# lebrice/blurred-GAN

Hardware: AMD Instinct MI355X
Metric: images/sec (G+D+GP step) (higher is better)
Workload: dtype f32; 1 GPU; celeba64 64x64x3 batch 256/GPU, blur sigma 5.0 (31 taps), D-step+GP+G-step+Adam; global_batch=256, parallelism=dp1

## Files before the change

blurred-gan_amd/csrc/conv_rows.hip:

```cpp
#include "conv_common.h"
#include <algorithm>
#include <cstdlib>
#include <cstring>
#include <type_traits>

namespace {

typedef float floatx4 __attribute__((ext_vector_type(4)));

struct RowParams {
  const float* A;
  const float* Wt;
  float* C;
  int B, Hi, Wi, Ck, Ho, Wo, N;
  int pt, pl, flip;
  int R, strips;
  int wpr, ipw;
  int epi_mode;
  const float* bias;
  const float* ref;
  const unsigned char* keep;
  size_t keep_elems;
  float alpha, scale;
};

__device__ inline int floordiv(int a, int b) { return a >= 0 ? a / b : -((-a + b - 1) / b); }

__device__ inline float tanh_branchless(float x) {
  float ax = fabsf(x);
  ax = ax > 15.f ? 15.f : ax;
  const float e = __builtin_amdgcn_exp2f(ax * 2.885390081777927f);
  const float big = 1.f - 2.f * __builtin_amdgcn_rcpf(e + 1.f);
  const float x2 = ax * ax;
  const float small = ax * fmaf(x2, fmaf(x2, fmaf(x2, -17.f / 315.f, 2.f / 15.f), -1.f / 3.f), 1.f);
  return copysignf(ax < 0.1f ? small : big, x);
}

template <int KS, int K, int S, int PIXW, int EP>
__global__ __launch_bounds__(PIXW * 4) void conv_rows_scatter_kernel(const RowParams p) {
  constexpr int NTH = PIXW * 4;
  constexpr unsigned kOob = 0x80000000u;
  extern __shared__ __attribute__((aligned(16))) float row_lds[];
  constexpr int AS = 4 * KS + 4;
  float* abuf = row_lds;
  constexpr int PS = PIXW * 17 + 1;
  float* pbuf = row_lds + 2 * PIXW * AS;
  const int tid = threadIdx.x, lane = tid & 63, wave = tid >> 6;
  const int li = lane & 15, kq = lane >> 4;
  const int t = wave % p.wpr, img = wave / p.wpr;
  const int strip = blockIdx.x % p.strips, bgrp = blockIdx.x / p.strips;
  const int Ck = 4 * KS, N = p.N;
  const int y0 = strip * p.R, y1 = min(y0 + p.R, p.Ho);
  const int iy_lo = -floordiv(-(y0 + p.pt - (K - 1)), S);
  const int iy_hi = floordiv(y1 - 1 + p.pt, S);
  const int nrows = iy_hi - iy_lo + 1;
  const int nimg = min(p.ipw, p.B - bgrp * p.ipw);
  const size_t img0 = (size_t)bgrp * p.ipw;
  const __amdgpu_buffer_rsrc_t rsA = __builtin_amdgcn_make_buffer_rsrc(const_cast<float*>(p.A + img0 * p.Hi * p.Wi * Ck), 0,
                                                                        nimg * p.Hi * p.Wi * Ck * 4, 0x00020000);
  const __amdgpu_buffer_rsrc_t rsC = __builtin_amdgcn_make_buffer_rsrc(p.C + img0 * p.Ho * p.Wo * N, 0, nimg * p.Ho * p.Wo * N * 4, 0x00020000);

  float bw[K][KS];
  {
    const int lc = min(li, K * N - 1);
    const int kw = lc / N, n = lc - kw * N;
#pragma unroll
    for (int kh = 0; kh < K; ++kh) {
      const int tap = p.flip ? (K - 1 - kh) * K + (K - 1 - kw) : kh * K + kw;
#pragma unroll
      for (int ks = 0; ks < KS; ++ks) {
        const float w = p.Wt[((size_t)tap * N + n) * Ck + 4 * ks + kq];
        bw[kh][ks] = li < K * N ? w : 0.f;
      }
    }
  }
  floatx4 acc[K];
#pragma unroll
  for (int i = 0; i < K; ++i) acc[i] = floatx4{0.f, 0.f, 0.f, 0.f};

  constexpr int QPR = KS;
  constexpr int NQ = PIXW * QPR / NTH;
  static_assert(NQ >= 1, "Ck >= 16");
  unsigned g_off[NQ], l_off[NQ];
#pragma unroll
  for (int q = 0; q < NQ; ++q) {
    const int f = tid + q * NTH, pix = f / QPR, c4 = f - pix * QPR;
    const int im = pix / p.Wi, ix = pix - im * p.Wi;
    g_off[q] = im < nimg ? (unsigned)(((im * p.Hi * p.Wi + ix) * Ck + c4 * 4) * 4) : kOob;
    l_off[q] = (unsigned)(pix * AS + c4 * 4);
  }
  const int rowB = p.Wi * Ck * 4;
  auto gload = [&](int r, float4 (&g)[NQ]) {
    const int iy = iy_lo + r;
    const bool row_ok = r < nrows && (unsigned)iy < (unsigned)p.Hi;
    const unsigned add = row_ok ? (unsigned)(iy * rowB) : 0u, force = row_ok ? 0u : kOob;
#pragma unroll
    for (int q = 0; q < NQ; ++q)
      g[q] = __builtin_bit_cast(float4, __builtin_amdgcn_raw_buffer_load_b128(rsA, (g_off[q] + add) | force, 0, 0));
  };
  auto lstore = [&](int buf, const float4 (&g)[NQ]) {
#pragma unroll
    for (int q = 0; q < NQ; ++q) *reinterpret_cast<float4*>(abuf + (size_t)buf * PIXW * AS + l_off[q]) = g[q];
  };
  const float* afrag = abuf + ((size_t)img * p.Wi + 16 * t + li) * AS + kq;
  constexpr int NE = (S * (16 / K) + 3) / 4;
  constexpr int NTERM = (K + S - 1) / S;
  int e_src[NE][NTERM];
  unsigned e_dst[NE];
  float e_bias[NE], e_mul[NE];
  int e_n[NE];
  if (tid < 2 * S) pbuf[(size_t)tid * PS + PIXW * 17] = 0.f;
  {
    const int per_img = p.Wo * N;
#pragma unroll
    for (int q = 0; q < NE; ++q) {
      const int e = tid + q * NTH;
      const int im = e / per_img, rem = e - im * per_img;
      const int x = rem / N, n = rem - x * N;
      const bool ok = e < p.ipw * per_img && im < nimg;
      e_dst[q] = ok ? (unsigned)(((im * p.Ho * p.Wo + x) * N + n) * 4) : kOob;
      e_n[q] = n;
      e_bias[q] = ok && p.bias ? p.bias[n] : 0.f;
      e_mul[q] = ok && p.epi_mode == BG_EPI_AFFINE_LRELU ? p.ref[n] : 0.f;
#pragma unroll
      for (int i = 0; i < NTERM; ++i) {
        const int kw = (x + p.pl) % S + i * S;
        const int num = x + p.pl - kw, ix = num / S;
        e_src[q][i] = (ok && kw < K && num >= 0 && ix < p.Wi) ? (im * p.Wi + ix) * 17 + kw * N + n : PIXW * 17;
      }
    }
  }
  const size_t out0 = img0 * p.Ho * p.Wo * N;
  auto pwrite = [&](const floatx4& pacc, int slot) {
    float* pb = pbuf + (size_t)slot * PS;
#pragma unroll
    for (int rr = 0; rr < 4; ++rr) pb[((size_t)img * p.Wi + 16 * t + 4 * kq + rr) * 17 + li] = pacc[rr];
  };
  auto pstore = [&](int slot, int y, bool live) {
    const float* pb = pbuf + (size_t)slot * PS;
    float v[NE];
#pragma unroll
    for (int q = 0; q < NE; ++q) {
      v[q] = pb[e_src[q][0]];
#pragma unroll
      for (int i = 1; i < NTERM; ++i) v[q] += pb[e_src[q][i]];
    }
    const unsigned add = live ? (unsigned)(y * p.Wo * N * 4) : 0u, force = live ? 0u : kOob;
#pragma unroll
    for (int q = 0; q < NE; ++q) {
      const unsigned off = (e_dst[q] + add) | force;
      float o;
      if (EP == 0) {
        o = v[q] + e_bias[q];
      } else if (EP == 1) {
        o = tanh_branchless(v[q] + e_bias[q]);
      } else {
        const bool mine = (off & kOob) == 0;
        o = mine ? bg::apply_epilogue_pre(p, v[q], out0 + (off >> 2), e_bias[q], e_mul[q]) : 0.f;
      }
      __builtin_amdgcn_raw_buffer_store_b32(__builtin_bit_cast(unsigned, o), rsC, off, 0, 0);
    }
  };

  float4 g0[NQ], g1[NQ], g2[NQ], g3[NQ];
  gload(0, g0);
  gload(1, g1);
  gload(2, g2);
  gload(3, g3);
  lstore(0, g0);
  gload(4, g0);
#pragma unroll
  for (int i = 0; i < 4 * NE * S; ++i) __builtin_amdgcn_raw_buffer_store_b32(0u, rsC, kOob + 4u * i, 0, 0);
  int y_prev = 0;
  bool have_prev = false;
  auto flush_prev = [&](int prev_par) {
#pragma unroll
    for (int kh = 0; kh < S; ++kh) {
      const int y = y_prev + kh;
      pstore(prev_par * S + kh, y, have_prev & (y >= y0) & (y < y1));
    }
  };
  auto trip = [&](int r, auto parity, float4 (&g)[NQ]) {
    constexpr int cur = decltype(parity)::value;
    __syncthreads();
    float a[KS];
#pragma unroll
    for (int ks = 0; ks < KS; ++ks) a[ks] = afrag[(size_t)cur * PIXW * AS + 4 * ks];
#pragma unroll
    for (int ks = 0; ks < KS; ++ks)
#pragma unroll
      for (int kh = 0; kh < K; ++kh) acc[kh] = __builtin_amdgcn_mfma_f32_16x16x4f32(a[ks], bw[kh][ks], acc[kh], 0, 0, 0);
    flush_prev(cur ^ 1);
    lstore(cur ^ 1, g);
    gload(r + 5, g);
#pragma unroll
    for (int kh = 0; kh < S; ++kh) pwrite(acc[kh], cur * S + kh);
    y_prev = (iy_lo + r) * S - p.pt;
    have_prev = true;
#pragma unroll
    for (int i = 0; i < K; ++i) acc[i] = i + S < K ? acc[i + S] : floatx4{0.f, 0.f, 0.f, 0.f};
  };
  int r = 0;
  for (; r + 4 <= nrows; r += 4) {
    trip(r, std::integral_constant<int, 0>{}, g1);
    trip(r + 1, std::integral_constant<int, 1>{}, g2);
    trip(r + 2, std::integral_constant<int, 0>{}, g3);
    trip(r + 3, std::integral_constant<int, 1>{}, g0);
  }
  int last_par = 1;
  if (r < nrows) {
    trip(r, std::integral_constant<int, 0>{}, g1);
    last_par = 0;
    if (r + 1 < nrows) {
      trip(r + 1, std::integral_constant<int, 1>{}, g2);
      last_par = 1;
      if (r + 2 < nrows) {
        trip(r + 2, std::integral_constant<int, 0>{}, g3);
        last_par = 0;
      }
    }
  }
  __syncthreads();
  if (last_par == 0) flush_prev(0); else flush_prev(1);
}

template <int K, int S>
int launch_rows(const RowParams& p, dim3 grid, size_t lds, hipStream_t s) {
  const bool wide = p.Wi == 128;
  const int ep = p.epi_mode == BG_EPI_NONE ? 0 : p.epi_mode == BG_EPI_TANH ? 1 : 2;
#define BG_RS2(KSv, EPv) do { if (wide) bg::launch((conv_rows_scatter_kernel<KSv, K, S, 128, EPv>), grid, dim3(512), lds, s, p); \
                              else bg::launch((conv_rows_scatter_kernel<KSv, K, S, 64, EPv>), grid, dim3(256), lds, s, p); } while (0)
#define BG_RS(KSv) do { if (ep == 0) BG_RS2(KSv, 0); else if (ep == 1) BG_RS2(KSv, 1); else BG_RS2(KSv, 2); } while (0)
  switch (p.Ck) {
    case 16: BG_RS(4); return 1;
    case 32: BG_RS(8); return 1;
    case 64: BG_RS(16); return 1;
    default: return 0;
  }
#undef BG_RS
#undef BG_RS2
}

constexpr int kRgHalo = 16;

struct RowGParams {
  const float* A;
  const float* Wt;
  float* C;
  int B, Hi, Wi, Ct, Ho, Wo, N;
  int s, pt, pl, flip;
  int R, strips;
  int epi_mode;
  const float* bias;
  const float* ref;
  const unsigned char* keep;
  size_t keep_elems;
  float alpha, scale;
};

template <int TG, int NT, int K, bool MASK>
__global__ __launch_bounds__(256) void conv_rows_gather_kernel(const RowGParams p) {
  extern __shared__ __attribute__((aligned(16))) float xl[];
  const int tid = threadIdx.x, lane = tid & 63, wave = tid >> 6;
  const int li = lane & 15, kq = lane >> 4;
  const int Ct = p.Ct, N = 16 * NT, st = p.s;
  const int RS = p.Wi * Ct + 2 * kRgHalo;
  const int strip = blockIdx.x % p.strips, b = blockIdx.x / p.strips;
  const int oy0 = strip * p.R, rows = min(p.R, p.Ho - oy0);
  const int nrows_in = (rows - 1) * st + K;

  float bw[K][4][NT];
#pragma unroll
  for (int ks = 0; ks < 4; ++ks) {
    const int i = 4 * ks + kq, kw = i / Ct, ci = i - kw * Ct;
#pragma unroll
    for (int kh = 0; kh < K; ++kh) {
      const int tap = p.flip ? (K - 1 - kh) * K + (K - 1 - kw) : kh * K + kw;
#pragma unroll
      for (int nt = 0; nt < NT; ++nt) bw[kh][ks][nt] = i < K * Ct ? p.Wt[((size_t)tap * N + nt * 16 + li) * Ct + ci] : 0.f;
    }
  }
  const int RL = p.Wi * Ct;
  if ((RL & 3) == 0) {
    const int q4 = RS / 4;
    bg::stage_rows_f4<4>(xl, nrows_in, q4, RS, tid, [&](int r, int c4) -> const float* {
      const int iy = oy0 * st - p.pt + r, e = c4 * 4 - kRgHalo;
      return ((unsigned)iy < (unsigned)p.Hi && (unsigned)e < (unsigned)RL) ? p.A + ((size_t)b * p.Hi + iy) * RL + e : nullptr;
    });
  } else {
    for (int idx = tid; idx < nrows_in * RS; idx += 256) {
      const int r = idx / RS, c = idx - r * RS;
      const int iy = oy0 * st - p.pt + r, e = c - kRgHalo;
      float v = 0.f;
      if ((unsigned)iy < (unsigned)p.Hi && (unsigned)e < (unsigned)RL) v = p.A[((size_t)b * p.Hi + iy) * RL + e];
      xl[idx] = v;
    }
  }
  __syncthreads();

  float e_bias[NT], e_mul[NT];
#pragma unroll
  for (int nt = 0; nt < NT; ++nt) {
    e_bias[nt] = p.bias ? p.bias[nt * 16 + li] : 0.f;
    e_mul[nt] = p.epi_mode == BG_EPI_AFFINE_LRELU ? p.ref[nt * 16 + li] : 1.f;
  }
  const int groups = p.Wo / (16 * TG);
  const int nunits = rows * groups;
  for (int u = wave; u < nunits; u += 4) {
    const int r = u / groups, g = u - r * groups;
    const int oy = oy0 + r, ox0 = g * 16 * TG;
    floatx4 acc[TG][NT];
#pragma unroll
    for (int tg = 0; tg < TG; ++tg)
#pragma unroll
      for (int nt = 0; nt < NT; ++nt) acc[tg][nt] = floatx4{0.f, 0.f, 0.f, 0.f};
    const float* abase = xl + (size_t)(r * st) * RS + kRgHalo + ((ox0 + li) * st - p.pl) * Ct + kq;
#pragma unroll
    for (int kh = 0; kh < K; ++kh) {
      float a[TG][4];
#pragma unroll
      for (int tg = 0; tg < TG; ++tg)
#pragma unroll
        for (int ks = 0; ks < 4; ++ks) a[tg][ks] = abase[(size_t)kh * RS + tg * 16 * st * Ct + 4 * ks];
#pragma unroll
      for (int ks = 0; ks < 4; ++ks)
#pragma unroll
        for (int tg = 0; tg < TG; ++tg)
#pragma unroll
          for (int nt = 0; nt < NT; ++nt) acc[tg][nt] = __builtin_amdgcn_mfma_f32_16x16x4f32(a[tg][ks], bw[kh][ks][nt], acc[tg][nt], 0, 0, 0);
    }
    constexpr bool mask_epi = MASK;
#pragma unroll
    for (int tg = 0; tg < TG; ++tg) {
      const size_t pix0 = ((size_t)b * p.Ho + oy) * p.Wo + ox0 + 16 * tg + 4 * kq;
      unsigned char e_keep[4][NT];
      if (mask_epi) {
#pragma unroll
        for (int rr = 0; rr < 4; ++rr)
#pragma unroll
          for (int nt = 0; nt < NT; ++nt) {
            const size_t idx = (pix0 + rr) * N + nt * 16 + li;
            e_keep[rr][nt] = p.keep[(p.keep_elems == 0 || idx < p.keep_elems) ? idx : 0];
          }
      }
#pragma unroll
      for (int rr = 0; rr < 4; ++rr)
#pragma unroll
        for (int nt = 0; nt < NT; ++nt) {
          const size_t idx = (pix0 + rr) * N + nt * 16 + li;
          if (mask_epi) {
            float v = acc[tg][nt][rr] + e_bias[nt];
            v = v > 0.f ? v : p.alpha * v;
            if (p.keep_elems == 0 || idx < p.keep_elems) v = e_keep[rr][nt] ? v * p.scale : 0.f;
            p.C[idx] = v;
          } else {
            p.C[idx] = bg::apply_epilogue_pre(p, acc[tg][nt][rr], idx, e_bias[nt], e_mul[nt]);
          }
        }
    }
  }
}

template <int K>
int launch_rows_gather(const RowGParams& p, int tg, dim3 grid, size_t lds, hipStream_t s) {
  const int nt = p.N / 16;
  const bool mask = p.epi_mode == BG_EPI_BIAS_LRELU && p.keep != nullptr;
#define BG_RG(TGv, NTv) do { if (mask) bg::launch((conv_rows_gather_kernel<TGv, NTv, K, true>), grid, dim3(256), lds, s, p); \
                             else bg::launch((conv_rows_gather_kernel<TGv, NTv, K, false>), grid, dim3(256), lds, s, p); } while (0)
  if (tg == 1) { if (nt == 1) BG_RG(1, 1); else if (nt == 2) BG_RG(1, 2); else BG_RG(1, 4); }
  else if (tg == 2) { if (nt == 1) BG_RG(2, 1); else if (nt == 2) BG_RG(2, 2); else BG_RG(2, 4); }
  else { if (nt == 1) BG_RG(4, 1); else if (nt == 2) BG_RG(4, 2); else BG_RG(4, 4); }
#undef BG_RG
  return 1;
}

}

namespace bg {

int try_conv_rows_gather(int bwd_data, const float* a, const float* w, float* c, int B, int H, int W, int Cin, int Cout, int k, int s,
                         const bg_epilogue* epi, void* stream, int* taken) {
  *taken = 0;
  static const int off = getenv("BG_NO_ROWS") ? 1 : 0;
  if (off || (k != 5 && k != 3)) return BG_OK;
  RowGParams p;
  memset(&p, 0, sizeof p);
  int Ho, Wo, pt, pl;
  same_pads(H, k, s, &Ho, &pt);
  same_pads(W, k, s, &Wo, &pl);
  if (bwd_data) {
    if (s != 1 || Cout * k > 16 || (Cin != 16 && Cin != 32 && Cin != 64)) return BG_OK;
    p.Hi = H; p.Wi = W; p.Ct = Cout; p.Ho = H; p.Wo = W; p.N = Cin; p.s = 1; p.pt = k - 1 - pt; p.pl = k - 1 - pl; p.flip = 1;
  } else {
    if (Cin * k > 16 || (Cout != 16 && Cout != 32 && Cout != 64)) return BG_OK;
    p.Hi = H; p.Wi = W; p.Ct = Cin; p.Ho = Ho; p.Wo = Wo; p.N = Cout; p.s = s; p.pt = pt; p.pl = pl; p.flip = 0;
  }
  if (p.Wo % 16 != 0) return BG_OK;
  if ((size_t)B * p.Ho * p.Wo * p.N >= (1ull << 31)) return BG_OK;
  const int tiles = p.Wo / 16;
  const int tg = tiles % 4 == 0 ? 4 : (tiles % 2 == 0 ? 2 : 1);
  p.A = a; p.Wt = w; p.C = c; p.B = B;
  static const int rows_r = getenv("BG_ROWSG_R") ? atoi(getenv("BG_ROWSG_R")) : 0;
  p.R = std::min(rows_r ? rows_r : (s == 2 ? 8 : 16), p.Ho);
  p.strips = (int)cdiv(p.Ho, p.R);
  const size_t lds = ((size_t)((p.R - 1) * p.s + k) * (p.Wi * p.Ct + 2 * kRgHalo)) * sizeof(float);
  if (lds > 64 * 1024) return BG_OK;
  p.epi_mode = BG_EPI_NONE; p.alpha = 0.3f; p.scale = 1.f;
  if (epi) {
    BG_REQUIRE(epi->mode >= BG_EPI_NONE && epi->mode <= BG_EPI_AFFINE_LRELU, BG_ERR_UNSUPPORTED, "conv rows: epilogue mode %d", epi->mode);
    BG_REQUIRE(epi->mode != BG_EPI_MUL_GRAD || epi->ref, BG_ERR_NULL, "conv rows: BG_EPI_MUL_GRAD needs ref");
    BG_REQUIRE(epi->mode != BG_EPI_AFFINE_LRELU || (epi->ref && epi->bias), BG_ERR_NULL, "conv rows: BG_EPI_AFFINE_LRELU needs ref and bias");
    p.epi_mode = epi->mode; p.bias = epi->bias; p.ref = epi->ref; p.keep = epi->keep; p.keep_elems = epi->keep_elems; p.alpha = epi->alpha; p.scale = epi->scale;
  }
  const dim3 grid((unsigned)(B * p.strips));
  const double flops = 2.0 * B * (double)Ho * Wo * Cin * Cout * k * k;
  Launch L(stream, bwd_data ? "conv_rows_thin_k_dgrad" : "conv_rows_thin_k_fwd", flops, 0);
  if (k == 5) launch_rows_gather<5>(p, tg, grid, lds, L.s);
  else launch_rows_gather<3>(p, tg, grid, lds, L.s);
  *taken = 1;
  return L.done("conv_rows_gather_kernel");
}



int try_conv_rows(int bwd_data, const float* a, const float* w, float* c, int B, int H, int W, int Cin, int Cout, int k, int s,
                  const bg_epilogue* epi, void* stream, int* taken) {
  *taken = 0;
  static const int off = getenv("BG_NO_ROWS") ? 1 : 0;
  if (off || (k != 5 && k != 3)) return BG_OK;
  RowParams p;
  memset(&p, 0, sizeof p);
  int Ho, Wo, pt, pl;
  same_pads(H, k, s, &Ho, &pt);
  same_pads(W, k, s, &Wo, &pl);
  if (bwd_data) {
    if (Cin * k > 16 || (Cout != 16 && Cout != 32 && Cout != 64)) return BG_OK;
    p.Hi = Ho; p.Wi = Wo; p.Ck = Cout; p.Ho = H; p.Wo = W; p.N = Cin; p.pt = pt; p.pl = pl; p.flip = 0;
  } else {
    if (s != 1 || Cout * k > 16 || (Cin != 16 && Cin != 32 && Cin != 64)) return BG_OK;
    p.Hi = H; p.Wi = W; p.Ck = Cin; p.Ho = H; p.Wo = W; p.N = Cout; p.pt = k - 1 - pt; p.pl = k - 1 - pl; p.flip = 1;
  }
  if (p.Wi != 16 && p.Wi != 32 && p.Wi != 64 && p.Wi != 128) return BG_OK;
  if ((size_t)B * p.Hi * p.Wi * p.Ck >= (1ull << 31) || (size_t)B * p.Ho * p.Wo * p.N >= (1ull << 31)) return BG_OK;
  p.A = a; p.Wt = w; p.C = c; p.B = B;
  static const int rows_r = getenv("BG_ROWS_R") ? atoi(getenv("BG_ROWS_R")) : 0;
  p.R = std::min(rows_r ? rows_r : (s == 1 ? 32 : 16), p.Ho);
  p.strips = (int)cdiv(p.Ho, p.R);
  p.wpr = p.Wi / 16;
  p.ipw = p.Wi == 128 ? 1 : 4 / p.wpr;
  const int pixw = p.Wi == 128 ? 128 : 64;
  if ((long)p.ipw * p.Wo * p.N > (long)((s * (16 / k) + 3) / 4) * pixw * 4) return BG_OK;
  if ((size_t)p.ipw * p.Hi * p.Wi * p.Ck >= (1ull << 29) || (size_t)p.ipw * p.Ho * p.Wo * p.N >= (1ull << 29)) return BG_OK;
  p.epi_mode = BG_EPI_NONE; p.alpha = 0.3f; p.scale = 1.f;
  if (epi) {
    BG_REQUIRE(epi->mode >= BG_EPI_NONE && epi->mode <= BG_EPI_AFFINE_LRELU, BG_ERR_UNSUPPORTED, "conv rows: epilogue mode %d", epi->mode);
    BG_REQUIRE(epi->mode != BG_EPI_MUL_GRAD || epi->ref, BG_ERR_NULL, "conv rows: BG_EPI_MUL_GRAD needs ref");
    BG_REQUIRE(epi->mode != BG_EPI_AFFINE_LRELU || (epi->ref && epi->bias), BG_ERR_NULL, "conv rows: BG_EPI_AFFINE_LRELU needs ref and bias");
    p.epi_mode = epi->mode; p.bias = epi->bias; p.ref = epi->ref; p.keep = epi->keep; p.keep_elems = epi->keep_elems; p.alpha = epi->alpha; p.scale = epi->scale;
  }
  const dim3 grid((unsigned)(cdiv(B, p.ipw) * p.strips));
  const size_t lds = ((size_t)2 * pixw * (p.Ck + 4) + (size_t)2 * s * (pixw * 17 + 1)) * sizeof(float);
  const double flops = 2.0 * B * (double)H * W * Cin * Cout * k * k / (s * s);
  Launch L(stream, bwd_data ? "conv_rows_dgrad" : "conv_rows_fwd", flops, 0);
  int ok;
  if (k == 5) ok = s == 2 ? launch_rows<5, 2>(p, grid, lds, L.s) : launch_rows<5, 1>(p, grid, lds, L.s);
  else ok = s == 2 ? launch_rows<3, 2>(p, grid, lds, L.s) : launch_rows<3, 1>(p, grid, lds, L.s);
  (void)ok;
  *taken = 1;
  return L.done("conv_rows_scatter_kernel");
}

}
```

Baseline: 32460 images/s.

## Make thin-K row-gather conv persistent with double-buffered register prefetch

Turns the row-gather conv kernel into a persistent kernel sized to a few workgroups per CU. It prefetches the next strip's input rows into registers via buffer loads and stashes them into a second LDS buffer while the current strip computes. It also swaps the MFMA operand order so each lane holds four consecutive channels, which allows float4 epilogue stores and uchar4 keep-mask loads. The cost is doubled LDS, smaller default strips, added alignment requirements and register pressure from the prefetch arrays.

```diff
diff --git a/blurred-gan_amd/csrc/conv_rows.hip b/blurred-gan_amd/csrc/conv_rows.hip
--- a/blurred-gan_amd/csrc/conv_rows.hip
+++ b/blurred-gan_amd/csrc/conv_rows.hip
@@ -242,6 +242,8 @@
 }
 
 constexpr int kRgHalo = 16;
+constexpr int kRgPF = 6;
+constexpr int kRgWgPerCu = 3;
 
 struct RowGParams {
   const float* A;
@@ -250,6 +252,9 @@
   int B, Hi, Wi, Ct, Ho, Wo, N;
   int s, pt, pl, flip;
   int R, strips;
+  int units;
+  int vec;
+  unsigned a_bytes;
   int epi_mode;
   const float* bias;
   const float* ref;
@@ -261,13 +266,15 @@
 template <int TG, int NT, int K, bool MASK>
 __global__ __launch_bounds__(256) void conv_rows_gather_kernel(const RowGParams p) {
   extern __shared__ __attribute__((aligned(16))) float xl[];
+  constexpr unsigned kOob = 0x80000000u;
   const int tid = threadIdx.x, lane = tid & 63, wave = tid >> 6;
   const int li = lane & 15, kq = lane >> 4;
   const int Ct = p.Ct, N = 16 * NT, st = p.s;
-  const int RS = p.Wi * Ct + 2 * kRgHalo;
-  const int strip = blockIdx.x % p.strips, b = blockIdx.x / p.strips;
-  const int oy0 = strip * p.R, rows = min(p.R, p.Ho - oy0);
-  const int nrows_in = (rows - 1) * st + K;
+  const int RL = p.Wi * Ct;
+  const int RS = RL + 2 * kRgHalo;
+  const int nrows_in = (p.R - 1) * st + K;
+  const int BUF = nrows_in * RS;
+  const __amdgpu_buffer_rsrc_t rsA = __builtin_amdgcn_make_buffer_rsrc(const_cast<float*>(p.A), 0, (int)p.a_bytes, 0x00020000);
 
   float bw[K][4][NT];
 #pragma unroll
@@ -280,84 +287,140 @@
       for (int nt = 0; nt < NT; ++nt) bw[kh][ks][nt] = i < K * Ct ? p.Wt[((size_t)tap * N + nt * 16 + li) * Ct + ci] : 0.f;
     }
   }
-  const int RL = p.Wi * Ct;
-  if ((RL & 3) == 0) {
-    const int q4 = RS / 4;
-    bg::stage_rows_f4<4>(xl, nrows_in, q4, RS, tid, [&](int r, int c4) -> const float* {
-      const int iy = oy0 * st - p.pt + r, e = c4 * 4 - kRgHalo;
-      return ((unsigned)iy < (unsigned)p.Hi && (unsigned)e < (unsigned)RL) ? p.A + ((size_t)b * p.Hi + iy) * RL + e : nullptr;
-    });
-  } else {
-    for (int idx = tid; idx < nrows_in * RS; idx += 256) {
-      const int r = idx / RS, c = idx - r * RS;
-      const int iy = oy0 * st - p.pt + r, e = c - kRgHalo;
-      float v = 0.f;
-      if ((unsigned)iy < (unsigned)p.Hi && (unsigned)e < (unsigned)RL) v = p.A[((size_t)b * p.Hi + iy) * RL + e];
-      xl[idx] = v;
-    }
-  }
+  for (int i = tid; i < 2 * nrows_in * 2 * kRgHalo; i += 256) {
+    const int row = i / (2 * kRgHalo), e = i - row * (2 * kRgHalo);
+    xl[(size_t)row * RS + (e < kRgHalo ? e : RL + e)] = 0.f;
+  }
+  const int per_row = p.vec ? RL / 4 : RL;
+  const int tot = nrows_in * per_row;
+  const int npf = (tot + 255) / 256;
+  int pf_row[kRgPF], pf_g[kRgPF], pf_l[kRgPF];
+#pragma unroll
+  for (int i = 0; i < kRgPF; ++i) {
+    const int idx = tid + i * 256, r = idx / per_row, c = idx - r * per_row;
+    pf_row[i] = idx < tot ? r : -(1 << 24);
+    pf_g[i] = (r * RL + (p.vec ? 4 * c : c)) * 4;
+    pf_l[i] = r * RS + kRgHalo + (p.vec ? 4 * c : c);
+  }
+  float4 pf[kRgPF];
+  auto prefetch = [&](int unit) {
+    const int b = unit / p.strips, strip = unit - b * p.strips;
+    const int iy0 = strip * p.R * st - p.pt;
+    const bool live = unit < p.units;
+    const int base = (b * p.Hi + iy0) * RL * 4;
+    auto off = [&](int i) {
+      const bool ok = live && (unsigned)(iy0 + pf_row[i]) < (unsigned)p.Hi;
+      return ok ? (unsigned)(base + pf_g[i]) : kOob;
+    };
+    if (p.vec) {
+#pragma unroll
+      for (int i = 0; i < kRgPF / 2; ++i) pf[i] = __builtin_bit_cast(float4, __builtin_amdgcn_raw_buffer_load_b128(rsA, off(i), 0, 0));
+      if (npf > kRgPF / 2) {
+#pragma unroll
+        for (int i = kRgPF / 2; i < kRgPF; ++i) pf[i] = __builtin_bit_cast(float4, __builtin_amdgcn_raw_buffer_load_b128(rsA, off(i), 0, 0));
+      }
+    } else {
+#pragma unroll
+      for (int i = 0; i < kRgPF / 2; ++i) pf[i].x = __builtin_bit_cast(float, __builtin_amdgcn_raw_buffer_load_b32(rsA, off(i), 0, 0));
+      if (npf > kRgPF / 2) {
+#pragma unroll
+        for (int i = kRgPF / 2; i < kRgPF; ++i) pf[i].x = __builtin_bit_cast(float, __builtin_amdgcn_raw_buffer_load_b32(rsA, off(i), 0, 0));
+      }
+    }
+  };
+  auto stash = [&](int buf) {
+    float* dst = xl + (size_t)buf * BUF;
+    if (p.vec) {
+#pragma unroll
+      for (int i = 0; i < kRgPF; ++i)
+        if (pf_row[i] >= 0) *reinterpret_cast<float4*>(dst + pf_l[i]) = pf[i];
+    } else {
+#pragma unroll
+      for (int i = 0; i < kRgPF; ++i)
+        if (pf_row[i] >= 0) dst[pf_l[i]] = pf[i].x;
+    }
+  };
+
+  float4 e_bias[NT], e_mul[NT];
+#pragma unroll
+  for (int nt = 0; nt < NT; ++nt) {
+    const int n = nt * 16 + 4 * kq;
+    e_bias[nt] = p.bias ? *reinterpret_cast<const float4*>(p.bias + n) : make_float4(0.f, 0.f, 0.f, 0.f);
+    e_mul[nt] = p.epi_mode == BG_EPI_AFFINE_LRELU ? *reinterpret_cast<const float4*>(p.ref + n) : make_float4(1.f, 1.f, 1.f, 1.f);
+  }
+  const int groups = p.Wo / (16 * TG);
+
+  int unit = blockIdx.x;
+  prefetch(unit);
+  __builtin_amdgcn_s_waitcnt(0x0F70);
+  stash(0);
   __syncthreads();
-
-  float e_bias[NT], e_mul[NT];
-#pragma unroll
-  for (int nt = 0; nt < NT; ++nt) {
-    e_bias[nt] = p.bias ? p.bias[nt * 16 + li] : 0.f;
-    e_mul[nt] = p.epi_mode == BG_EPI_AFFINE_LRELU ? p.ref[nt * 16 + li] : 1.f;
-  }
-  const int groups = p.Wo / (16 * TG);
-  const int nunits = rows * groups;
-  for (int u = wave; u < nunits; u += 4) {
-    const int r = u / groups, g = u - r * groups;
-    const int oy = oy0 + r, ox0 = g * 16 * TG;
-    floatx4 acc[TG][NT];
-#pragma unroll
-    for (int tg = 0; tg < TG; ++tg)
-#pragma unroll
-      for (int nt = 0; nt < NT; ++nt) acc[tg][nt] = floatx4{0.f, 0.f, 0.f, 0.f};
-    const float* abase = xl + (size_t)(r * st) * RS + kRgHalo + ((ox0 + li) * st - p.pl) * Ct + kq;
-#pragma unroll
-    for (int kh = 0; kh < K; ++kh) {
-      float a[TG][4];
+  for (int buf = 0; unit < p.units; unit += gridDim.x, buf ^= 1) {
+    prefetch(unit + gridDim.x);
+    const int b = unit / p.strips, strip = unit - b * p.strips;
+    const int oy0 = strip * p.R, rows = min(p.R, p.Ho - oy0);
+    const int nunits = rows * groups;
+    const float* xb = xl + (size_t)buf * BUF;
+    if (wave >= nunits) stash(buf ^ 1);
+    for (int u = wave; u < nunits; u += 4) {
+      const int r = u / groups, g = u - r * groups;
+      const int oy = oy0 + r, ox0 = g * 16 * TG;
+      floatx4 acc[TG][NT];
 #pragma unroll
       for (int tg = 0; tg < TG; ++tg)
 #pragma unroll
-        for (int ks = 0; ks < 4; ++ks) a[tg][ks] = abase[(size_t)kh * RS + tg * 16 * st * Ct + 4 * ks];
-#pragma unroll
-      for (int ks = 0; ks < 4; ++ks)
+        for (int nt = 0; nt < NT; ++nt) acc[tg][nt] = floatx4{0.f, 0.f, 0.f, 0.f};
+      const float* abase = xb + (size_t)(r * st) * RS + kRgHalo + ((ox0 + li) * st - p.pl) * Ct + kq;
+#pragma unroll
+      for (int kh = 0; kh < K; ++kh) {
+        float a[TG][4];
 #pragma unroll
         for (int tg = 0; tg < TG; ++tg)
 #pragma unroll
-          for (int nt = 0; nt < NT; ++nt) acc[tg][nt] = __builtin_amdgcn_mfma_f32_16x16x4f32(a[tg][ks], bw[kh][ks][nt], acc[tg][nt], 0, 0, 0);
-    }
-    constexpr bool mask_epi = MASK;
-#pragma unroll
-    for (int tg = 0; tg < TG; ++tg) {
-      const size_t pix0 = ((size_t)b * p.Ho + oy) * p.Wo + ox0 + 16 * tg + 4 * kq;
-      unsigned char e_keep[4][NT];
+          for (int ks = 0; ks < 4; ++ks) a[tg][ks] = abase[(size_t)kh * RS + tg * 16 * st * Ct + 4 * ks];
+#pragma unroll
+        for (int ks = 0; ks < 4; ++ks)
+#pragma unroll
+          for (int tg = 0; tg < TG; ++tg)
+#pragma unroll
+            for (int nt = 0; nt < NT; ++nt) acc[tg][nt] = __builtin_amdgcn_mfma_f32_16x16x4f32(bw[kh][ks][nt], a[tg][ks], acc[tg][nt], 0, 0, 0);
+      }
+      if (u + 4 >= nunits) stash(buf ^ 1);
+      constexpr bool mask_epi = MASK;
+      const size_t pix0 = ((size_t)b * p.Ho + oy) * p.Wo + ox0 + li;
+      uchar4 e_keep[TG][NT];
       if (mask_epi) {
 #pragma unroll
-        for (int rr = 0; rr < 4; ++rr)
+        for (int tg = 0; tg < TG; ++tg)
 #pragma unroll
           for (int nt = 0; nt < NT; ++nt) {
-            const size_t idx = (pix0 + rr) * N + nt * 16 + li;
-            e_keep[rr][nt] = p.keep[(p.keep_elems == 0 || idx < p.keep_elems) ? idx : 0];
+            const size_t idx = (pix0 + 16 * tg) * N + nt * 16 + 4 * kq;
+            e_keep[tg][nt] = *reinterpret_cast<const uchar4*>(p.keep + ((p.keep_elems == 0 || idx < p.keep_elems) ? idx : 0));
           }
       }
 #pragma unroll
-      for (int rr = 0; rr < 4; ++rr)
+      for (int tg = 0; tg < TG; ++tg)
 #pragma unroll
         for (int nt = 0; nt < NT; ++nt) {
-          const size_t idx = (pix0 + rr) * N + nt * 16 + li;
+          const size_t idx = (pix0 + 16 * tg) * N + nt * 16 + 4 * kq;
+          float4 v = make_float4(acc[tg][nt][0], acc[tg][nt][1], acc[tg][nt][2], acc[tg][nt][3]);
           if (mask_epi) {
-            float v = acc[tg][nt][rr] + e_bias[nt];
-            v = v > 0.f ? v : p.alpha * v;
-            if (p.keep_elems == 0 || idx < p.keep_elems) v = e_keep[rr][nt] ? v * p.scale : 0.f;
-            p.C[idx] = v;
+            const float4 bb = e_bias[nt];
+            const uchar4 k = e_keep[tg][nt];
+            v.x += bb.x; v.y += bb.y; v.z += bb.z; v.w += bb.w;
+            v.x = v.x > 0.f ? v.x : p.alpha * v.x; v.y = v.y > 0.f ? v.y : p.alpha * v.y;
+            v.z = v.z > 0.f ? v.z : p.alpha * v.z; v.w = v.w > 0.f ? v.w : p.alpha * v.w;
+            if (p.keep_elems == 0 || idx + 0 < p.keep_elems) v.x = k.x ? v.x * p.scale : 0.f;
+            if (p.keep_elems == 0 || idx + 1 < p.keep_elems) v.y = k.y ? v.y * p.scale : 0.f;
+            if (p.keep_elems == 0 || idx + 2 < p.keep_elems) v.z = k.z ? v.z * p.scale : 0.f;
+            if (p.keep_elems == 0 || idx + 3 < p.keep_elems) v.w = k.w ? v.w * p.scale : 0.f;
           } else {
-            p.C[idx] = bg::apply_epilogue_pre(p, acc[tg][nt][rr], idx, e_bias[nt], e_mul[nt]);
+            v = bg::apply_epilogue4(p, v, idx, reinterpret_cast<const float*>(&e_bias[nt]), reinterpret_cast<const float*>(&e_mul[nt]));
           }
+          *reinterpret_cast<float4*>(p.C + idx) = v;
         }
     }
+    __syncthreads();
   }
 }
 
@@ -401,18 +464,34 @@
   const int tg = tiles % 4 == 0 ? 4 : (tiles % 2 == 0 ? 2 : 1);
   p.A = a; p.Wt = w; p.C = c; p.B = B;
   static const int rows_r = getenv("BG_ROWSG_R") ? atoi(getenv("BG_ROWSG_R")) : 0;
-  p.R = std::min(rows_r ? rows_r : (s == 2 ? 8 : 16), p.Ho);
+  const size_t a_bytes = (size_t)B * p.Hi * p.Wi * p.Ct * sizeof(float);
+  if (a_bytes >= (1ull << 31)) return BG_OK;
+  p.a_bytes = (unsigned)a_bytes;
+  p.vec = (p.Wi * p.Ct) % 4 == 0;
+  p.R = std::min(rows_r ? rows_r : 8, p.Ho);
+  size_t lds = 0;
+  for (;; p.R /= 2) {
+    const size_t rows_in = (size_t)(p.R - 1) * p.s + k, row_items = p.vec ? p.Wi * p.Ct / 4 : p.Wi * p.Ct;
+    lds = 2 * rows_in * (p.Wi * p.Ct + 2 * kRgHalo) * sizeof(float);
+    if (rows_in * row_items <= (size_t)kRgPF * 256 && lds <= 64 * 1024) break;
+    if (p.R == 1) return BG_OK;
+  }
   p.strips = (int)cdiv(p.Ho, p.R);
-  const size_t lds = ((size_t)((p.R - 1) * p.s + k) * (p.Wi * p.Ct + 2 * kRgHalo)) * sizeof(float);
-  if (lds > 64 * 1024) return BG_OK;
+  p.units = B * p.strips;
   p.epi_mode = BG_EPI_NONE; p.alpha = 0.3f; p.scale = 1.f;
   if (epi) {
     BG_REQUIRE(epi->mode >= BG_EPI_NONE && epi->mode <= BG_EPI_AFFINE_LRELU, BG_ERR_UNSUPPORTED, "conv rows: epilogue mode %d", epi->mode);
     BG_REQUIRE(epi->mode != BG_EPI_MUL_GRAD || epi->ref, BG_ERR_NULL, "conv rows: BG_EPI_MUL_GRAD needs ref");
     BG_REQUIRE(epi->mode != BG_EPI_AFFINE_LRELU || (epi->ref && epi->bias), BG_ERR_NULL, "conv rows: BG_EPI_AFFINE_LRELU needs ref and bias");
+    if (!bg::aligned16(epi->bias) || !bg::aligned16(epi->ref) || (reinterpret_cast<uintptr_t>(epi->keep) & 3u) != 0 || epi->keep_elems % 4 != 0) return BG_OK;
     p.epi_mode = epi->mode; p.bias = epi->bias; p.ref = epi->ref; p.keep = epi->keep; p.keep_elems = epi->keep_elems; p.alpha = epi->alpha; p.scale = epi->scale;
   }
-  const dim3 grid((unsigned)(B * p.strips));
+  static const int cus = [] {
+    int dev = 0, n = 0;
+    if (hipGetDevice(&dev) != hipSuccess || hipDeviceGetAttribute(&n, hipDeviceAttributeMultiprocessorCount, dev) != hipSuccess || n <= 0) n = 256;
+    return n;
+  }();
+  const dim3 grid((unsigned)std::min(p.units, cus * kRgWgPerCu));
   const double flops = 2.0 * B * (double)Ho * Wo * Cin * Cout * k * k;
   Launch L(stream, bwd_data ? "conv_rows_thin_k_dgrad" : "conv_rows_thin_k_fwd", flops, 0);
   if (k == 5) launch_rows_gather<5>(p, tg, grid, lds, L.s);
```

Result: no change. 32540 images/s, median of 6 (+0.3%).
